# teofum/rust_raytracer

Hardware: AMD Instinct MI355X
Metric: Msamples/sec (whole node), cornell_dragon 870k tri @1000spp (higher is better)
Workload: dtype f64; 1 GPU; scenes/cornell_dragon 1200x1200 @1000spp (10 replicas x 10x10 strata), 871200-tri stand-in mesh; spp=1000, seed=1, pipeline=auto, frames_in_flight=1, partition=1200-row bands round-robin over 1 GPU(s)

## Files before the change

### rust_raytracer_amd/csrc/rt_bvh.cpp

```cpp
#include "rt_bvh.h"

#include <algorithm>
#include <cmath>
#include <cstdlib>
#include <limits>

#include "rt_refit.h"
#include "rt_scene.h"

namespace rt {
namespace {

constexpr int kMaxBins = 64;
static int g_bins = 16;
constexpr double kInf = std::numeric_limits<double>::infinity();

struct Box {
    double lo[3] = {kInf, kInf, kInf};
    double hi[3] = {-kInf, -kInf, -kInf};
    void grow(const double* p) {
        for (int a = 0; a < 3; a++) {
            if (p[a] < lo[a]) lo[a] = p[a];
            if (p[a] > hi[a]) hi[a] = p[a];
        }
// ... 228 lines not shown
Bvh4Build collapse_bvh4(const BvhBuild& b2) { return collapse<4>(b2); }



ConeLimits cone_limits(bool f32) {
    if (f32) return ConeLimits{1.0 / 32.0, 1e-12, 1e12};
    return ConeLimits{1.0 / 1048576.0, 1e-100, 1e100};
}

void build_mesh_cones(const std::vector<BuildNode4>& nodes4, const std::vector<TriRec<double>>& tris, const ConeLimits& lim,
                      std::vector<uint32_t>* out) {
    const size_t n_tris = tris.size();
    std::vector<double> normal(3 * n_tris);
    const double kNaN = std::numeric_limits<double>::quiet_NaN();
    for (size_t t = 0; t < n_tris; t++) rf_tri_normal(tris[t].v0, tris[t].e1, tris[t].e2, lim, &normal[3 * t]);
    struct Below {
        uint32_t lo = UINT32_MAX, hi = 0, count = 0;
        double sum[3] = {0.0, 0.0, 0.0};
        void add(const Below& o) {
            lo = std::min(lo, o.lo); hi = std::max(hi, o.hi); count += o.count;
            for (int a = 0; a < 3; a++) sum[a] += o.sum[a];
        }
    };
    auto cone_word = [&](const Below& b) -> uint32_t { return rf_cone_word(normal.data(), b.lo, b.hi, b.count, b.sum); };
    out->assign(4 * nodes4.size(), kNeutralCone);
    std::vector<Below> below(nodes4.size());
    for (size_t i = nodes4.size(); i-- > 0;) {
        const BuildNode4& nd = nodes4[i];
        Below all;
        for (int k = 0; k < 4; k++) {
            const int32_t ch = nd.child[k];
            if (ch == kEmptyChild) continue;
            Below b;
            if (ch >= 0) {
                if (size_t(ch) <= i || size_t(ch) >= nodes4.size()) { all.sum[0] = kNaN; continue; }
                b = below[size_t(ch)];
            } else {
                const uint32_t code = uint32_t(~ch), first = code >> 3, count = (code & 7u) + 1u;
                if (size_t(first) + count > n_tris) { all.sum[0] = kNaN; continue; }
                b.lo = first; b.hi = first + count; b.count = count;
                for (uint32_t t = first; t < first + count; t++)
                    for (int a = 0; a < 3; a++) b.sum[a] += normal[3 * size_t(t) + a];
            }
            (*out)[4 * i + size_t(k)] = cone_word(b);
            all.add(b);
        }
        below[i] = all;
    }
}

void build_mesh_slabs(const std::vector<BuildNode4>& nodes4, const std::vector<TriRec<double>>& tris, const std::vector<uint32_t>& cones,
                      const BvhNode4q* qnodes, const double* node_pad, std::vector<uint32_t>* out) {
    const size_t n_tris = tris.size();
    struct Run { uint32_t lo = UINT32_MAX, hi = 0, count = 0; };
    auto tri_at = [&](uint32_t t, double* v) {
        const TriRec<double>& r = tris[t];
        for (int a = 0; a < 3; a++) { v[a] = r.v0[a]; v[3 + a] = r.e1[a]; v[6 + a] = r.e2[a]; }
    };
    out->assign(4 * nodes4.size(), kNeutralSlab);
    std::vector<Run> below(nodes4.size());
    for (size_t i = nodes4.size(); i-- > 0;) {
        const BuildNode4& nd = nodes4[i];
        Run all;
        for (int k = 0; k < 4; k++) {
            const int32_t ch = nd.child[k];
            if (ch == kEmptyChild) continue;
            Run b;
            if (ch >= 0) {
                if (size_t(ch) <= i || size_t(ch) >= nodes4.size()) continue;
                b = below[size_t(ch)];
            } else {
                const uint32_t code = uint32_t(~ch), first = code >> 3, count = (code & 7u) + 1u;
                if (size_t(first) + count > n_tris) continue;
                b.lo = first; b.hi = first + count; b.count = count;
            }
            (*out)[4 * i + size_t(k)] = rf_slab_word(cones[4 * i + size_t(k)], qnodes[i].org, qnodes[i].cell, node_pad[i], b.lo, b.hi, b.count, tri_at);
            all.lo = std::min(all.lo, b.lo); all.hi = std::max(all.hi, b.hi);
            all.count += b.count;
        }
        below[i] = all;
    }
}

}
```

### rust_raytracer_amd/csrc/rt_bvh.h

```cpp
#pragma once
#include <cstdint>
#include <string>
#include <vector>

#include "rt_scene.h"

namespace rt {

struct BuildNode {
    double lo0[3], hi0[3], lo1[3], hi1[3];
    int32_t c0, c1;
};

struct BvhBuild {
    std::vector<BuildNode> nodes;
    std::vector<uint32_t> tri_order;
    uint32_t max_depth = 0;
};

BvhBuild build_bvh(const double* positions, const uint32_t* tri_pos, uint32_t n_tris, uint32_t max_leaf);

bool build_bvh_device(const double* positions, uint32_t n_positions, const uint32_t* tri_pos, uint32_t n_tris, uint32_t max_leaf,
                      BvhBuild* out, std::string* err);

template <int W>
struct BuildNodeN {
    double lo[W][3], hi[W][3];
    int32_t child[W];
};
template <int W>
struct BvhNBuild {
    std::vector<BuildNodeN<W>> nodes;
    uint32_t max_depth = 0;
    uint32_t max_stack = 0;
    double root_lo[3], root_hi[3];
};
using BuildNode4 = BuildNodeN<4>;
using Bvh4Build = BvhNBuild<4>;
Bvh4Build collapse_bvh4(const BvhBuild& bvh2);

struct ConeLimits {
    double sigma;
    double min_edge;
    double max_edge;
};
ConeLimits cone_limits(bool f32);
void build_mesh_cones(const std::vector<BuildNode4>& nodes4, const std::vector<TriRec<double>>& tris, const ConeLimits& lim,
                      std::vector<uint32_t>* out);
void build_mesh_slabs(const std::vector<BuildNode4>& nodes4, const std::vector<TriRec<double>>& tris, const std::vector<uint32_t>& cones,
                      const BvhNode4q* qnodes, const double* node_pad, std::vector<uint32_t>* out);

}
```

### rust_raytracer_amd/csrc/rt_refit.h

```cpp
#pragma once
#include <cmath>
#include <cstdint>
#include <cstring>
#include <limits>
#include <string>
#include <vector>

#include "../../include/rt_mi355.h"
#include "rt_bvh.h"
#include "rt_scene.h"

#if defined(__HIP__)
#include <hip/hip_runtime.h>

#include "rt_owned.h"
#define RT_HD __host__ __device__
#else
#define RT_HD
#endif

namespace rt {

RT_HD inline double rf_min(double a, double b) { return b < a ? b : a; }
RT_HD inline double rf_max(double a, double b) { return b > a ? b : a; }
// ... 85 lines not shown
            uint32_t ql = 255u, qh = 0u;
            if (any && real[k]) {
                const double l = std::floor((flo[k] - org) / cell), h = std::ceil((fhi[k] - org) / cell);
                const double lc = 255.0 < l ? 255.0 : l, hc = 255.0 < h ? 255.0 : h;
                ql = uint32_t(0.0 < lc ? lc : 0.0);
                qh = uint32_t(0.0 < hc ? hc : 0.0);
                if (!(org + ql * cell <= flo[k] && org + qh * cell >= fhi[k])) return false;
            }
            qlo[a] |= ql << (8 * k);
            qhi[a] |= qh << (8 * k);
        }
    }
    return true;
}

constexpr double kConeDirSlack = 0.00682;
constexpr double kConeSafety = 0.001;
constexpr double kConeMinCos = 0.125;

RT_HD inline void rf_tri_normal(const double* v0, const double* a, const double* b, const ConeLimits& lim, double* out) {
    const double cx = a[1] * b[2] - a[2] * b[1], cy = a[2] * b[0] - a[0] * b[2], cz = a[0] * b[1] - a[1] * b[0];
    const double la = std::sqrt(a[0] * a[0] + a[1] * a[1] + a[2] * a[2]), lb = std::sqrt(b[0] * b[0] + b[1] * b[1] + b[2] * b[2]);
    const double lc = std::sqrt(cx * cx + cy * cy + cz * cz);
    bool ok = std::isfinite(v0[0]) && std::isfinite(v0[1]) && std::isfinite(v0[2]);
    ok = ok && la >= lim.min_edge && la <= lim.max_edge && lb >= lim.min_edge && lb <= lim.max_edge;
    ok = ok && lc >= lim.sigma * la * lb && lc > 0.0;
    const double kNaN = std::numeric_limits<double>::quiet_NaN();
    out[0] = ok ? cx / lc : kNaN;
    out[1] = ok ? cy / lc : kNaN;
    out[2] = ok ? cz / lc : kNaN;
}

RT_HD inline uint32_t rf_cone_around(const double* normal, uint32_t lo, uint32_t hi, const double* axis) {
    const double l = std::sqrt(axis[0] * axis[0] + axis[1] * axis[1] + axis[2] * axis[2]);
    if (!(l > 0.0) || !std::isfinite(l)) return kNeutralCone;
    int q[3];
    double al = 0.0;
    for (int a = 0; a < 3; a++) { q[a] = int(std::lround(127.0 * axis[a] / l)); al += double(q[a]) * double(q[a]); }
    al = std::sqrt(al);
    if (!(al > 0.0)) return kNeutralCone;
    const double ax = q[0] / al, ay = q[1] / al, az = q[2] / al;
    double c = 1.0;
    for (uint32_t t = lo; t < hi; t++) {
        const double d = ax * normal[3 * size_t(t)] + ay * normal[3 * size_t(t) + 1] + az * normal[3 * size_t(t) + 2];
        c = d < c ? d : c;
        if (c < kConeMinCos) return kNeutralCone;
    }
    if (!(c >= kConeMinCos)) return kNeutralCone;
    const double s = std::sqrt(std::fmax(0.0, 1.0 - c * c));
    const double w = std::ceil(al * (s + kConeDirSlack + kConeSafety));
    if (!(w >= 1.0 && w <= 127.0)) return kNeutralCone;
    return uint32_t(q[0] & 0xFF) | (uint32_t(q[1] & 0xFF) << 8) | (uint32_t(q[2] & 0xFF) << 16) | (uint32_t(w) << 24);
}

RT_HD inline uint32_t rf_cone_word(const double* normal, uint32_t lo, uint32_t hi, uint32_t count, const double* sum) {
    if (count == 0 || hi - lo != count) return kNeutralCone;
    uint32_t word = rf_cone_around(normal, lo, hi, sum);
    if (word == kNeutralCone && count >= 2 && count <= 8 && std::isfinite(sum[0])) {
        uint32_t bi = lo, bj = lo;
        double least = 2.0;
        for (uint32_t i = lo; i < hi; i++)
            for (uint32_t j = i + 1; j < hi; j++) {
                const double* ni = &normal[3 * size_t(i)];
                const double* nj = &normal[3 * size_t(j)];
                const double dij = ni[0] * nj[0] + ni[1] * nj[1] + ni[2] * nj[2];
                if (dij < least) { least = dij; bi = i; bj = j; }
            }
        const double mid[3] = {normal[3 * size_t(bi)] + normal[3 * size_t(bj)], normal[3 * size_t(bi) + 1] + normal[3 * size_t(bj) + 1],
                               normal[3 * size_t(bi) + 2] + normal[3 * size_t(bj) + 2]};
        word = rf_cone_around(normal, lo, hi, mid);
    }
    return word;
}

RT_HD inline double rf_slab_inv_scale(const float* cell) {
    const double cmax = rf_max(double(cell[0]), rf_max(double(cell[1]), double(cell[2])));
    return 0.25 / cmax;
}
RT_HD inline double rf_slab_margin(const int* q, double pad, double inv_s) {
    const double l1 = double((q[0] < 0 ? -q[0] : q[0]) + (q[1] < 0 ? -q[1] : q[1]) + (q[2] < 0 ? -q[2] : q[2]));
    return l1 * (2.0 * pad * inv_s + 1.0 / 4096.0);
}

template <typename TriAt>
RT_HD inline uint32_t rf_slab_word(uint32_t cone, const float* org, const float* cell, double pad, uint32_t lo, uint32_t hi, uint32_t count, TriAt tri_at) {
    if (cone == kNeutralCone || count == 0 || hi - lo != count) return kNeutralSlab;
    const int q[3] = {int(int8_t(cone & 0xFFu)), int(int8_t((cone >> 8) & 0xFFu)), int(int8_t((cone >> 16) & 0xFFu))};
    const double inv_s = rf_slab_inv_scale(cell);
    if (!(inv_s > 0.0) || !std::isfinite(inv_s) || !std::isfinite(pad)) return kNeutralSlab;
    double plo = INFINITY, phi = -INFINITY;
    for (uint32_t t = lo; t < hi; t++) {
        double v[9];
        tri_at(t, v);
        for (int c = 0; c < 3; c++) {
            double x[3];
            for (int a = 0; a < 3; a++) x[a] = c == 0 ? v[a] : v[a] + v[3 * c + a];
            const double p = double(q[0]) * ((x[0] - double(org[0])) * inv_s) + double(q[1]) * ((x[1] - double(org[1])) * inv_s) +
                             double(q[2]) * ((x[2] - double(org[2])) * inv_s);
            plo = rf_min(plo, p);
            phi = rf_max(phi, p);
        }
    }
    if (!(plo <= phi) || !std::isfinite(plo) || !std::isfinite(phi)) return kNeutralSlab;
    const double margin = rf_slab_margin(q, pad, inv_s);
    const double l = rf_max(std::floor(plo - margin), -32768.0), h = rf_min(std::ceil(phi + margin), 32767.0);
    if (!(l <= 32767.0 && h >= -32768.0)) return kNeutralSlab;
    return (uint32_t(int32_t(l)) & 0xFFFFu) | (uint32_t(int32_t(h)) << 16);
}

#if defined(__HIP__)
struct RefitMesh {
    uint32_t n_tris = 0, n_nodes = 0, n_nodes4 = 0, n_positions = 0, n_normals = 0, n_uvs = 0;
    DevBuf<uint32_t> tri_order, tri_pos, tri_nrm;
    DevBuf<int32_t> tri_uv;
    DevBuf<int32_t> child2, child4;
    DevBuf<int32_t> parent2, parent4;
    DevBuf<uint32_t> inner2, inner4;
    DevBuf<uint32_t> arrived2, arrived4;
    DevBuf<double> positions, normals, uvs;
    DevBuf<double> tri_box, tri_normal;
    DevBuf<double> box2, box4;
    DevBuf<double> sum4;
    DevBuf<uint32_t> run4;
};

template <typename R>
struct RefitTarget {
    BvhNode<R>* nodes;
    BvhNode4f* nodes4;
    MeshNode4qc* nodes4q;
    TriRec<R>* tris;
    TriAttr<R>* attrs;
    double pad4;
};

bool refit_mesh_upload(RefitMesh& rm, const RtMesh& m, const uint32_t* tri_order, const int32_t* child2, uint32_t n_nodes, const int32_t* child4,
                       uint32_t n_nodes4, hipStream_t stream, uint64_t* bytes, std::string* err);
template <typename R> bool refit_mesh_launch(RefitMesh& rm, const RefitTarget<R>& t, hipStream_t stream, std::string* err);
#endif

}
```

### rust_raytracer_amd/csrc/rt_refit.hip

```cpp
#include "rt_refit.h"

#include <algorithm>

namespace rt {
namespace {

#define REFIT_TRY(expr)                                                                 \
    do {                                                                                \
        hipError_t e_ = (expr);                                                         \
        if (e_ != hipSuccess) {                                                         \
            *err = std::string("scene refit: ") + hipGetErrorString(e_) + " at " #expr; \
            return false;                                                               \
        }                                                                               \
    } while (0)

template <typename R>
__global__ void k_refit_tris(uint32_t n, const uint32_t* __restrict__ tri_order, const uint32_t* __restrict__ tri_pos,
                             const uint32_t* __restrict__ tri_nrm, const int32_t* __restrict__ tri_uv, const double* __restrict__ positions,
                             const double* __restrict__ normals, const double* __restrict__ uvs, ConeLimits lim, TriRec<R>* __restrict__ tris,
                             TriAttr<R>* __restrict__ attrs, double* __restrict__ tri_box, double* __restrict__ tri_normal) {
    const uint32_t slot = blockIdx.x * blockDim.x + threadIdx.x;
    if (slot >= n) return;
    const size_t t = tri_order[slot];
    const double* p0 = positions + 3 * size_t(tri_pos[3 * t]);
// ... 82 lines not shown
        if (W == 4) {
            for (int a = 0; a < 3; a++) sum[3 * (W * size_t(i) + k) + a] = s[a];
            run[3 * (W * size_t(i) + k)] = rlo; run[3 * (W * size_t(i) + k) + 1] = rhi; run[3 * (W * size_t(i) + k) + 2] = cnt;
        }
    }
}

template <int W>
__global__ void k_refit_up(uint32_t n_nodes, uint32_t n_tris, const int32_t* __restrict__ child, const int32_t* __restrict__ parent,
                           const uint32_t* __restrict__ inner, unsigned int* __restrict__ arrived, const double* __restrict__ tri_box,
                           const double* __restrict__ tri_normal, double* box, double* sum, uint32_t* run) {
    const uint32_t first = blockIdx.x * blockDim.x + threadIdx.x;
    if (first >= n_nodes || inner[first] != 0u) return;
    int32_t node = int32_t(first);
    for (uint32_t guard = 0; guard <= n_nodes; guard++) {
        refit_node<W>(uint32_t(node), n_nodes, n_tris, child, tri_box, tri_normal, box, sum, run);
        __threadfence();
        const int32_t up = parent[node];
        if (up < 0 || uint32_t(up) >= n_nodes) return;
        if (atomicAdd(&arrived[up], 1u) + 1u < inner[up]) return;
        __threadfence();
        node = up;
    }
}

template <typename R>
__global__ void k_refit_nodes2(uint32_t n_nodes, const double* __restrict__ box, BvhNode<R>* __restrict__ nodes) {
    const uint32_t i = blockIdx.x * blockDim.x + threadIdx.x;
    if (i >= n_nodes) return;
    BvhNode<R>& n = nodes[i];
    const double* b0 = box + 12 * size_t(i);
    const double* b1 = b0 + 6;
    for (int a = 0; a < 3; a++) {
        rf_pad_box2<R>(b0[a], b0[3 + a], &n.lo0[a], &n.hi0[a]);
        rf_pad_box2<R>(b1[a], b1[3 + a], &n.lo1[a], &n.hi1[a]);
    }
}

__global__ void k_refit_nodes4(uint32_t n_nodes, double pad, const int32_t* __restrict__ child, const double* __restrict__ box,
                               const double* __restrict__ sum, const uint32_t* __restrict__ run, const double* __restrict__ tri_normal,
                               const uint32_t* __restrict__ tri_order, const uint32_t* __restrict__ tri_pos, const double* __restrict__ positions,
                               BvhNode4f* __restrict__ nodes4, MeshNode4qc* __restrict__ nodes4q) {
    const uint32_t i = blockIdx.x * blockDim.x + threadIdx.x;
    if (i >= n_nodes) return;
    double lo[4][3], hi[4][3];
    int32_t ch[4];
    for (int k = 0; k < 4; k++) {
        ch[k] = child[4 * size_t(i) + k];
        for (int a = 0; a < 3; a++) { lo[k][a] = box[6 * (4 * size_t(i) + k) + a]; hi[k][a] = box[6 * (4 * size_t(i) + k) + 3 + a]; }
    }
    BvhNode4f& f = nodes4[i];
    for (int k = 0; k < 4; k++) {
        rf_pad_box4f(lo[k][0], hi[k][0], pad, &f.lox[k], &f.hix[k]);
        rf_pad_box4f(lo[k][1], hi[k][1], pad, &f.loy[k], &f.hiy[k]);
        rf_pad_box4f(lo[k][2], hi[k][2], pad, &f.loz[k], &f.hiz[k]);
    }
    float org[3] = {0.f, 0.f, 0.f}, cell[3] = {0.f, 0.f, 0.f};
    uint32_t qlo[3], qhi[3];
    MeshNode4qc& q = nodes4q[i];
    if (rf_quantise4(lo, hi, ch, pad, org, cell, qlo, qhi))
        for (int a = 0; a < 3; a++) { q.node.org[a] = org[a]; q.node.cell[a] = cell[a]; q.node.qlo[a] = qlo[a]; q.node.qhi[a] = qhi[a]; }
    for (int k = 0; k < 4; k++) {
        uint32_t word = kNeutralCone;
        if (ch[k] != kEmptyChild) {
            const uint32_t* r = run + 3 * (4 * size_t(i) + k);
            word = rf_cone_word(tri_normal, r[0], r[1], r[2], sum + 3 * (4 * size_t(i) + k));
        }
        q.cones.word[k] = word;
        uint32_t slab = kNeutralSlab;
        if (word != kNeutralCone) {
            const uint32_t* r = run + 3 * (4 * size_t(i) + k);
            slab = rf_slab_word(word, org, cell, pad, r[0], r[1], r[2], [&](uint32_t slot, double* v) {
                const size_t t = tri_order[slot];
                const double* p0 = positions + 3 * size_t(tri_pos[3 * t]);
                const double* p1 = positions + 3 * size_t(tri_pos[3 * t + 1]);
                const double* p2 = positions + 3 * size_t(tri_pos[3 * t + 2]);
                for (int a = 0; a < 3; a++) { v[a] = p0[a]; v[3 + a] = p1[a] - p0[a]; v[6 + a] = p2[a] - p0[a]; }
            });
        }
        q.slabs.word[k] = slab;
    }
}

template <typename T>
bool dev_alloc(DevBuf<T>& p, size_t n, std::string* err) {
    if (p.reserve(std::max<size_t>(n, 1) * sizeof(T)) == RT_OK) return true;
    *err = "scene refit: " + g_err;
    return false;
}
template <typename T>
bool dev_put(DevBuf<T>& dst, const T* src, size_t n, hipStream_t stream, uint64_t* bytes, std::string* err) {
    if (n) REFIT_TRY(hipMemcpyAsync(dst, src, n * sizeof(T), hipMemcpyHostToDevice, stream));
    *bytes += n * sizeof(T);
    return true;
}

inline dim3 grid_for(uint32_t n) { return dim3((n + 255u) / 256u); }

}

bool refit_mesh_upload(RefitMesh& rm, const RtMesh& m, const uint32_t* tri_order, const int32_t* child2, uint32_t n_nodes, const int32_t* child4,
                       uint32_t n_nodes4, hipStream_t stream, uint64_t* bytes, std::string* err) {
    if (!rm.tri_order) {
        RefitMesh r;
        r.n_tris = m.n_triangles; r.n_nodes = n_nodes; r.n_nodes4 = n_nodes4;
        r.n_positions = m.n_positions; r.n_normals = m.n_normals; r.n_uvs = m.uvs && m.tri_uv ? m.n_uvs : 0;
        const size_t nt = r.n_tris;
        bool ok = dev_alloc(r.tri_order, nt, err) && dev_alloc(r.tri_pos, 3 * nt, err) && dev_alloc(r.tri_nrm, 3 * nt, err) &&
                  (!m.tri_uv || dev_alloc(r.tri_uv, 3 * nt, err)) && dev_alloc(r.child2, 2 * size_t(n_nodes), err) &&
                  dev_alloc(r.child4, 4 * size_t(n_nodes4), err) && dev_alloc(r.parent2, n_nodes, err) && dev_alloc(r.parent4, n_nodes4, err) &&
                  dev_alloc(r.inner2, n_nodes, err) && dev_alloc(r.inner4, n_nodes4, err) && dev_alloc(r.arrived2, n_nodes, err) &&
                  dev_alloc(r.arrived4, n_nodes4, err) && dev_alloc(r.positions, 3 * size_t(r.n_positions), err) &&
                  dev_alloc(r.normals, 3 * size_t(r.n_normals), err) && (!r.n_uvs || dev_alloc(r.uvs, 3 * size_t(r.n_uvs), err)) &&
                  dev_alloc(r.tri_box, 6 * nt, err) && dev_alloc(r.tri_normal, 3 * nt, err) && dev_alloc(r.box2, 12 * size_t(n_nodes), err) &&
                  dev_alloc(r.box4, 24 * size_t(n_nodes4), err) && dev_alloc(r.sum4, 12 * size_t(n_nodes4), err) &&
                  dev_alloc(r.run4, 12 * size_t(n_nodes4), err);
        ok = ok && dev_put(r.tri_order, tri_order, nt, stream, bytes, err) && dev_put(r.tri_pos, m.tri_pos, 3 * nt, stream, bytes, err) &&
             dev_put(r.tri_nrm, m.tri_nrm, 3 * nt, stream, bytes, err) && (!m.tri_uv || dev_put(r.tri_uv, m.tri_uv, 3 * nt, stream, bytes, err)) &&
             dev_put(r.child2, child2, 2 * size_t(n_nodes), stream, bytes, err) && dev_put(r.child4, child4, 4 * size_t(n_nodes4), stream, bytes, err);
        if (!ok) return false;
        hipLaunchKernelGGL(k_refit_parents<2>, grid_for(n_nodes), dim3(256), 0, stream, n_nodes, r.child2.get(), r.parent2.get(), r.inner2.get());
        hipLaunchKernelGGL(k_refit_parents<4>, grid_for(n_nodes4), dim3(256), 0, stream, n_nodes4, r.child4.get(), r.parent4.get(), r.inner4.get());
        hipError_t e = hipGetLastError();
        if (e == hipSuccess) e = hipStreamSynchronize(stream);
        if (e != hipSuccess) { *err = std::string("scene refit: ") + hipGetErrorString(e); return false; }
        rm = std::move(r);
    }
    if (rm.n_tris != m.n_triangles || rm.n_positions != m.n_positions || rm.n_normals != m.n_normals || rm.n_nodes != n_nodes || rm.n_nodes4 != n_nodes4) {
        *err = "scene refit: the mesh has another structure than at its first update";
        return false;
    }
    return dev_put(rm.positions, m.positions, 3 * size_t(rm.n_positions), stream, bytes, err) &&
           dev_put(rm.normals, m.normals, 3 * size_t(rm.n_normals), stream, bytes, err) &&
           (!rm.n_uvs || dev_put(rm.uvs, m.uvs, 3 * size_t(rm.n_uvs), stream, bytes, err));
}

template <typename R>
bool refit_mesh_launch(RefitMesh& rm, const RefitTarget<R>& t, hipStream_t stream, std::string* err) {
    if (rm.n_tris == 0) return true;
    const dim3 block(256);
    REFIT_TRY(hipMemsetAsync(rm.arrived2, 0, size_t(rm.n_nodes) * sizeof(uint32_t), stream));
    REFIT_TRY(hipMemsetAsync(rm.arrived4, 0, size_t(rm.n_nodes4) * sizeof(uint32_t), stream));
    hipLaunchKernelGGL((k_refit_tris<R>), grid_for(rm.n_tris), block, 0, stream, rm.n_tris, rm.tri_order.get(), rm.tri_pos.get(), rm.tri_nrm.get(), rm.uvs ? rm.tri_uv.get() : nullptr,
                       rm.positions.get(), rm.normals.get(), rm.uvs.get(), cone_limits(sizeof(R) == 4), t.tris, t.attrs, rm.tri_box.get(), rm.tri_normal.get());
    hipLaunchKernelGGL((k_refit_up<2>), grid_for(rm.n_nodes), block, 0, stream, rm.n_nodes, rm.n_tris, rm.child2.get(), rm.parent2.get(), rm.inner2.get(), rm.arrived2.get(),
                       rm.tri_box.get(), rm.tri_normal.get(), rm.box2.get(), static_cast<double*>(nullptr), static_cast<uint32_t*>(nullptr));
    hipLaunchKernelGGL((k_refit_up<4>), grid_for(rm.n_nodes4), block, 0, stream, rm.n_nodes4, rm.n_tris, rm.child4.get(), rm.parent4.get(), rm.inner4.get(), rm.arrived4.get(),
                       rm.tri_box.get(), rm.tri_normal.get(), rm.box4.get(), rm.sum4.get(), rm.run4.get());
    hipLaunchKernelGGL((k_refit_nodes2<R>), grid_for(rm.n_nodes), block, 0, stream, rm.n_nodes, rm.box2.get(), t.nodes);
    hipLaunchKernelGGL(k_refit_nodes4, grid_for(rm.n_nodes4), block, 0, stream, rm.n_nodes4, t.pad4, rm.child4.get(), rm.box4.get(), rm.sum4.get(), rm.run4.get(),
                       rm.tri_normal.get(), rm.tri_order.get(), rm.tri_pos.get(), rm.positions.get(), t.nodes4, t.nodes4q);
    REFIT_TRY(hipGetLastError());
    return true;
}
template bool refit_mesh_launch<float>(RefitMesh&, const RefitTarget<float>&, hipStream_t, std::string*);
template bool refit_mesh_launch<double>(RefitMesh&, const RefitTarget<double>&, hipStream_t, std::string*);

}
```

### rust_raytracer_amd/csrc/rt_tables.cpp

```cpp
#include "rt_tables.h"

#include <algorithm>
#include <cmath>

#include "rt_refit.h"

namespace rt {

static int refuse(std::string* err, const char* msg) {
    if (err) *err = msg;
    return RT_E_UNSUPPORTED;
}

double mesh_pad(const CompiledScene& cs, const CompiledScene::MeshGeom& g) {
    double pad = 0.0;
    for (size_t i = 0; i < cs.meshes.size(); i++)
        if (cs.meshes[i].node4_base == g.node4_base) pad = std::fmax(pad, rf_pad_of_box(cs.mesh_bounds[i].lo, cs.mesh_bounds[i].hi));
    return pad;
}

template <typename R> static void derive_nodes2(const CompiledScene& cs, std::vector<BvhNode<R>>* out) {
    out->resize(cs.nodes.size());
    for (size_t i = 0; i < out->size(); i++) {
        const BuildNode& s = cs.nodes[i];
        BvhNode<R>& n = (*out)[i];
        for (int a = 0; a < 3; a++) {
            rf_pad_box2<R>(s.lo0[a], s.hi0[a], &n.lo0[a], &n.hi0[a]);
            rf_pad_box2<R>(s.lo1[a], s.hi1[a], &n.lo1[a], &n.hi1[a]);
        }
        n.c0 = s.c0;
        n.c1 = s.c1;
    }
}

static std::vector<double> derive_node_pads(const CompiledScene& cs) {
    std::vector<double> pad(cs.nodes4.size(), 0.0);
    for (const CompiledScene::MeshGeom& g : cs.mesh_geoms) std::fill_n(pad.begin() + g.node4_base, g.n_nodes4, mesh_pad(cs, g));
    return pad;
}

static void derive_nodes4f(const CompiledScene& cs, const std::vector<double>& node_pad, std::vector<BvhNode4f>* out) {
    out->resize(cs.nodes4.size());
    for (size_t i = 0; i < out->size(); i++) {
        const BuildNode4& sn = cs.nodes4[i];
        BvhNode4f& dn = (*out)[i];
        for (int k = 0; k < 4; k++) {
            float* lo[3] = {&dn.lox[k], &dn.loy[k], &dn.loz[k]};
            float* hi[3] = {&dn.hix[k], &dn.hiy[k], &dn.hiz[k]};
            for (int a = 0; a < 3; a++) rf_pad_box4f(sn.lo[k][a], sn.hi[k][a], node_pad[i], lo[a], hi[a]);
            dn.child[k] = sn.child[k];
            dn._pad[k] = 0;
        }
    }
}

static bool quantise(const BuildNode4& sn, double m, BvhNode4q& qn) {
    for (int k = 0; k < 4; k++) qn.child[k] = sn.child[k];
    return rf_quantise4(sn.lo, sn.hi, sn.child, m, qn.org, qn.cell, qn.qlo, qn.qhi);
}

static int derive_nodes4qc(const CompiledScene& cs, const std::vector<double>& node_pad, bool f32, std::vector<MeshNode4qc>* out, std::string* err) {
    std::vector<BvhNode4q> nodes4q(cs.nodes4.size());
    for (size_t i = 0; i < nodes4q.size(); i++)
        if (!quantise(cs.nodes4[i], node_pad[i], nodes4q[i])) return refuse(err, "BVH node does not fit the 8-bit grid");
    std::vector<uint32_t> cone_words, slab_words;
    build_mesh_cones(cs.nodes4, cs.tris, cone_limits(f32), &cone_words);
    build_mesh_slabs(cs.nodes4, cs.tris, cone_words, nodes4q.data(), node_pad.data(), &slab_words);
    out->resize(cs.nodes4.size());
    for (size_t i = 0; i < out->size(); i++) {
        MeshNode4qc& n = (*out)[i];
        n.node = nodes4q[i];
        for (int k = 0; k < 4; k++) n.cones.word[k] = cone_words[4 * i + size_t(k)];
        for (int k = 0; k < 4; k++) n.slabs.word[k] = slab_words[4 * i + size_t(k)];
        for (uint32_t& x : n._pad) x = 0;
    }
    return RT_OK;
}

template <typename R> static void derive_triangles(const CompiledScene& cs, std::vector<TriRec<R>>* tris, std::vector<TriAttr<R>>* attrs) {
    tris->resize(cs.tris.size());
    for (size_t i = 0; i < tris->size(); i++) {
        TriRec<R>& t = (*tris)[i];
        cast_arr(t.v0, cs.tris[i].v0); cast_arr(t.e1, cs.tris[i].e1); cast_arr(t.e2, cs.tris[i].e2);
        t._pad = R(0);
    }
    attrs->resize(cs.attrs.size());
    for (size_t i = 0; i < attrs->size(); i++) {
        const auto& s = cs.attrs[i];
        TriAttr<R>& a = (*attrs)[i];
        cast_arr(a.n0, s.n0); cast_arr(a.n1, s.n1); cast_arr(a.n2, s.n2);
        cast_arr(a.uv0, s.uv0); cast_arr(a.uv1, s.uv1); cast_arr(a.uv2, s.uv2);
        a.has_uv = s.has_uv;
        a._pad = 0;
    }
}

template <typename R>
int derive_mesh_tables(const CompiledScene& cs, MeshTables<R>* out, std::string* err) {
    *out = MeshTables<R>{};
    const std::vector<double> node_pad = derive_node_pads(cs);
    derive_nodes2(cs, &out->nodes);
    derive_nodes4f(cs, node_pad, &out->nodes4);
    if (int st = derive_nodes4qc(cs, node_pad, sizeof(R) == 4, &out->nodes4qc, err)) return st;
    derive_triangles(cs, &out->tris, &out->attrs);
    return RT_OK;
}

template <typename R> static void derive_prims(const CompiledScene& cs, SceneTables<R>* t) {
    t->bounds.resize(cs.bounds.size());
    for (size_t i = 0; i < t->bounds.size(); i++) {
        cast_arr(t->bounds[i].lo, cs.bounds[i].lo);
        cast_arr(t->bounds[i].hi, cs.bounds[i].hi);
    }
    t->xforms.resize(cs.xforms.size());
    for (size_t i = 0; i < t->xforms.size(); i++) {
        cast_arr(t->xforms[i].m, cs.xforms[i].m);
        cast_arr(t->xforms[i].inv, cs.xforms[i].inv);
    }
    t->spheres.resize(cs.spheres.size());
    for (size_t i = 0; i < t->spheres.size(); i++) {
        cast_arr(t->spheres[i].center, cs.spheres[i].center);
        t->spheres[i].radius = R(cs.spheres[i].radius);
        t->spheres[i].material = cs.spheres[i].material;
        t->spheres[i]._pad = 0;
    }
    t->planes.resize(cs.planes.size());
    for (size_t i = 0; i < t->planes.size(); i++) {
        const auto& s = cs.planes[i];
        PlanePrim<R>& p = t->planes[i];
        cast_arr(p.corner, s.corner); cast_arr(p.normal, s.normal);
        cast_arr(p.u, s.u); cast_arr(p.v, s.v);
        cast_arr(p.inv_u, s.inv_u); cast_arr(p.inv_v, s.inv_v);
        p.area = R(s.area);
        p.material = s.material;
        p.backface = s.backface;
    }
    t->suns.resize(cs.suns.size());
    for (size_t i = 0; i < t->suns.size(); i++) {
        cast_arr(t->suns[i].direction, cs.suns[i].direction);
        t->suns[i].material = cs.suns[i].material;
        t->suns[i]._pad = 0;
    }
    t->volumes.resize(cs.volumes.size());
    for (size_t i = 0; i < t->volumes.size(); i++) {
        t->volumes[i].neg_inv_density = R(cs.volumes[i].neg_inv_density);
        t->volumes[i].material = cs.volumes[i].material;
        t->volumes[i]._pad = 0;
    }
}
// ... 124 lines not shown
```

Before: 1587 Msamples/s.

## Add oriented slab axes to BVH4 children lacking normal cones

For BVH4 child slots that have no usable normal cone, the build now projects the child's triangles onto 46 fixed oblique axes. It picks the axis whose extent is smallest relative to the AABB, and only if that ratio is below a threshold, then stores it as a slab-only word with a quantised slab interval. A matching GPU refit kernel recomputes the choice after refit. The aim is to cull more ray-box hits with a tighter oriented slab test, in exchange for extra build and refit work. The traversal code that consumes slab-only words is not shown here.

```diff
diff --git a/rust_raytracer_amd/csrc/rt_bvh.cpp b/rust_raytracer_amd/csrc/rt_bvh.cpp
--- a/rust_raytracer_amd/csrc/rt_bvh.cpp
+++ b/rust_raytracer_amd/csrc/rt_bvh.cpp
@@ -334,4 +334,121 @@
     }
 }
 
-}
+bool slab_axes_enabled() {
+    const char* e = std::getenv("RT_SLAB_AXES");
+    return !(e && *e && std::atoi(e) == 0);
+}
+
+namespace {
+struct AxisSupport {
+    double lo[kSlabAxes], hi[kSlabAxes];
+    AxisSupport() { for (int c = 0; c < kSlabAxes; c++) { lo[c] = INFINITY; hi[c] = -INFINITY; } }
+    void merge(const AxisSupport& o) { for (int c = 0; c < kSlabAxes; c++) { lo[c] = rf_min(lo[c], o.lo[c]); hi[c] = rf_max(hi[c], o.hi[c]); } }
+};
+
+struct AxisPass {
+    const std::vector<BuildNode4>& nodes4;
+    const std::vector<TriRec<double>>& tris;
+    const BvhNode4q* qnodes;
+    const double* node_pad;
+    std::vector<uint32_t>& cones;
+    struct Run { uint32_t lo = UINT32_MAX, hi = 0, count = 0; };
+    std::vector<Run> run;
+    std::vector<uint8_t> eligible;
+    std::vector<uint8_t> done;
+    double ax[kSlabAxes], ay[kSlabAxes], az[kSlabAxes];
+
+    void project(uint32_t lo, uint32_t hi, AxisSupport* s) const {
+        double mn[kSlabAxes], mx[kSlabAxes];
+        for (int c = 0; c < kSlabAxes; c++) { mn[c] = s->lo[c]; mx[c] = s->hi[c]; }
+        for (uint32_t t = lo; t < hi; t++) {
+            const TriRec<double>& r = tris[t];
+            double v[9];
+            for (int a = 0; a < 3; a++) { v[a] = r.v0[a]; v[3 + a] = r.e1[a]; v[6 + a] = r.e2[a]; }
+            for (int c3 = 0; c3 < 3; c3++) {
+                double x[3];
+                rf_tri_corner(v, c3, x);
+                const double x0 = x[0], x1 = x[1], x2 = x[2];
+                for (int c = 0; c < kSlabAxes; c++) {
+                    const double p = ax[c] * x0 + ay[c] * x1 + az[c] * x2;
+                    mn[c] = p < mn[c] ? p : mn[c];
+                    mx[c] = p > mx[c] ? p : mx[c];
+                }
+            }
+        }
+        for (int c = 0; c < kSlabAxes; c++) { s->lo[c] = mn[c]; s->hi[c] = mx[c]; }
+    }
+    void visit(size_t i, int k, AxisSupport* s) {
+        const size_t id = 4 * i + size_t(k), c = size_t(nodes4[i].child[k]);
+        done[id] = 1;
+        for (int j = 0; j < 4; j++) {
+            if (nodes4[c].child[j] == kEmptyChild) continue;
+            if (eligible[4 * c + size_t(j)]) {
+                AxisSupport below;
+                visit(c, j, &below);
+                s->merge(below);
+            } else {
+                project(run[4 * c + size_t(j)].lo, run[4 * c + size_t(j)].hi, s);
+            }
+        }
+        const int pick = rf_slab_axis_pick(nodes4[i].lo[k], nodes4[i].hi[k], s->lo, s->hi);
+        if (pick < 0) return;
+        const uint32_t word = rf_slab_axis_word(pick);
+        const Run& r = run[id];
+        const uint32_t slab = rf_slab_word(word, qnodes[i].org, qnodes[i].cell, node_pad[i], r.lo, r.hi, r.count, [&](uint32_t t, double* v) {
+            for (int a = 0; a < 3; a++) { v[a] = tris[t].v0[a]; v[3 + a] = tris[t].e1[a]; v[6 + a] = tris[t].e2[a]; }
+        });
+        if (slab != kNeutralSlab) cones[id] = word;
+    }
+};
+}
+
+void build_mesh_slab_axes(const std::vector<BuildNode4>& nodes4, const std::vector<TriRec<double>>& tris, const ConeLimits& lim,
+                          const BvhNode4q* qnodes, const double* node_pad, std::vector<uint32_t>* cones) {
+    const size_t n = nodes4.size(), n_tris = tris.size();
+    if (n == 0 || cones->size() != 4 * n) return;
+    AxisPass p{nodes4, tris, qnodes, node_pad, *cones, {}, {}, {}, {}, {}, {}};
+    for (int c = 0; c < kSlabAxes; c++) {
+        int q[3];
+        rf_slab_axis(c, q);
+        p.ax[c] = double(q[0]); p.ay[c] = double(q[1]); p.az[c] = double(q[2]);
+    }
+    std::vector<uint32_t> bad_before(n_tris + 1, 0);
+    for (size_t t = 0; t < n_tris; t++) {
+        double nrm[3];
+        rf_tri_normal(tris[t].v0, tris[t].e1, tris[t].e2, lim, nrm);
+        bad_before[t + 1] = bad_before[t] + (std::isfinite(nrm[0]) ? 0u : 1u);
+    }
+    p.run.resize(4 * n);
+    p.eligible.assign(4 * n, 0);
+    p.done.assign(4 * n, 0);
+    for (size_t i = n; i-- > 0;) {
+        for (int k = 0; k < 4; k++) {
+            const int32_t ch = nodes4[i].child[k];
+            AxisPass::Run& b = p.run[4 * i + size_t(k)];
+            if (ch == kEmptyChild) continue;
+            if (ch >= 0) {
+                if (size_t(ch) <= i || size_t(ch) >= n) continue;
+                for (int j = 0; j < 4; j++) {
+                    const AxisPass::Run& o = p.run[4 * size_t(ch) + size_t(j)];
+                    b.lo = std::min(b.lo, o.lo); b.hi = std::max(b.hi, o.hi); b.count += o.count;
+                }
+                if (b.count == 0 || b.hi - b.lo != b.count || b.hi > n_tris) continue;
+                const double clean[3] = {bad_before[b.hi] == bad_before[b.lo] ? 0.0 : std::numeric_limits<double>::quiet_NaN(), 0.0, 0.0};
+                p.eligible[4 * i + size_t(k)] = rf_slab_axis_eligible(0, 1, (*cones)[4 * i + size_t(k)], b.lo, b.hi, b.count, clean) ? 1 : 0;
+            } else {
+                const uint32_t code = uint32_t(~ch), first = code >> 3, count = (code & 7u) + 1u;
+                if (size_t(first) + count > n_tris) continue;
+                b.lo = first; b.hi = first + count; b.count = count;
+            }
+        }
+    }
+    for (size_t i = 0; i < n; i++)
+        for (int k = 0; k < 4; k++)
+            if (p.eligible[4 * i + size_t(k)] && !p.done[4 * i + size_t(k)]) {
+                AxisSupport s;
+                p.visit(i, k, &s);
+            }
+}
+
+}
diff --git a/rust_raytracer_amd/csrc/rt_bvh.h b/rust_raytracer_amd/csrc/rt_bvh.h
--- a/rust_raytracer_amd/csrc/rt_bvh.h
+++ b/rust_raytracer_amd/csrc/rt_bvh.h
@@ -47,6 +47,8 @@
 ConeLimits cone_limits(bool f32);
 void build_mesh_cones(const std::vector<BuildNode4>& nodes4, const std::vector<TriRec<double>>& tris, const ConeLimits& lim,
                       std::vector<uint32_t>* out);
+void build_mesh_slab_axes(const std::vector<BuildNode4>& nodes4, const std::vector<TriRec<double>>& tris, const ConeLimits& lim,
+                          const BvhNode4q* qnodes, const double* node_pad, std::vector<uint32_t>* cones);
 void build_mesh_slabs(const std::vector<BuildNode4>& nodes4, const std::vector<TriRec<double>>& tris, const std::vector<uint32_t>& cones,
                       const BvhNode4q* qnodes, const double* node_pad, std::vector<uint32_t>* out);
 
diff --git a/rust_raytracer_amd/csrc/rt_refit.h b/rust_raytracer_amd/csrc/rt_refit.h
--- a/rust_raytracer_amd/csrc/rt_refit.h
+++ b/rust_raytracer_amd/csrc/rt_refit.h
@@ -191,10 +191,29 @@
     return l1 * (2.0 * pad * inv_s + 1.0 / 4096.0);
 }
 
+RT_HD inline void rf_cone_axis(uint32_t cone, int* q) {
+    q[0] = int(int8_t(cone & 0xFFu)); q[1] = int(int8_t((cone >> 8) & 0xFFu)); q[2] = int(int8_t((cone >> 16) & 0xFFu));
+}
+RT_HD inline void rf_tri_corner(const double* v, int c, double* x) {
+    for (int a = 0; a < 3; a++) x[a] = c == 0 ? v[a] : v[a] + v[3 * c + a];
+}
+RT_HD inline double rf_slab_project(const int* q, const float* org, double inv_s, const double* x) {
+    return double(q[0]) * ((x[0] - double(org[0])) * inv_s) + double(q[1]) * ((x[1] - double(org[1])) * inv_s) +
+           double(q[2]) * ((x[2] - double(org[2])) * inv_s);
+}
+RT_HD inline uint32_t rf_slab_finish(const int* q, double pad, double inv_s, double plo, double phi) {
+    if (!(plo <= phi) || !std::isfinite(plo) || !std::isfinite(phi)) return kNeutralSlab;
+    const double margin = rf_slab_margin(q, pad, inv_s);
+    const double l = rf_max(std::floor(plo - margin), -32768.0), h = rf_min(std::ceil(phi + margin), 32767.0);
+    if (!(l <= 32767.0 && h >= -32768.0)) return kNeutralSlab;
+    return (uint32_t(int32_t(l)) & 0xFFFFu) | (uint32_t(int32_t(h)) << 16);
+}
+
 template <typename TriAt>
 RT_HD inline uint32_t rf_slab_word(uint32_t cone, const float* org, const float* cell, double pad, uint32_t lo, uint32_t hi, uint32_t count, TriAt tri_at) {
     if (cone == kNeutralCone || count == 0 || hi - lo != count) return kNeutralSlab;
-    const int q[3] = {int(int8_t(cone & 0xFFu)), int(int8_t((cone >> 8) & 0xFFu)), int(int8_t((cone >> 16) & 0xFFu))};
+    int q[3];
+    rf_cone_axis(cone, q);
     const double inv_s = rf_slab_inv_scale(cell);
     if (!(inv_s > 0.0) || !std::isfinite(inv_s) || !std::isfinite(pad)) return kNeutralSlab;
     double plo = INFINITY, phi = -INFINITY;
@@ -203,19 +222,74 @@
         tri_at(t, v);
         for (int c = 0; c < 3; c++) {
             double x[3];
-            for (int a = 0; a < 3; a++) x[a] = c == 0 ? v[a] : v[a] + v[3 * c + a];
-            const double p = double(q[0]) * ((x[0] - double(org[0])) * inv_s) + double(q[1]) * ((x[1] - double(org[1])) * inv_s) +
-                             double(q[2]) * ((x[2] - double(org[2])) * inv_s);
+            rf_tri_corner(v, c, x);
+            const double p = rf_slab_project(q, org, inv_s, x);
             plo = rf_min(plo, p);
             phi = rf_max(phi, p);
         }
     }
-    if (!(plo <= phi) || !std::isfinite(plo) || !std::isfinite(phi)) return kNeutralSlab;
-    const double margin = rf_slab_margin(q, pad, inv_s);
-    const double l = rf_max(std::floor(plo - margin), -32768.0), h = rf_min(std::ceil(phi + margin), 32767.0);
-    if (!(l <= 32767.0 && h >= -32768.0)) return kNeutralSlab;
-    return (uint32_t(int32_t(l)) & 0xFFFFu) | (uint32_t(int32_t(h)) << 16);
-}
+    return rf_slab_finish(q, pad, inv_s, plo, phi);
+}
+
+#ifndef RT_SLAB_AXIS_COUNT
+#define RT_SLAB_AXIS_COUNT 46
+#endif
+#ifndef RT_SLAB_AXIS_MAX_RATIO
+#define RT_SLAB_AXIS_MAX_RATIO 0.9
+#endif
+constexpr int kSlabAxes = RT_SLAB_AXIS_COUNT;
+static_assert(kSlabAxes >= 1 && kSlabAxes <= 46, "a prefix of the table");
+constexpr double kSlabAxisMaxRatio = RT_SLAB_AXIS_MAX_RATIO;
+RT_HD inline void rf_slab_axis(int c, int* q) {
+    static constexpr int8_t kTable[46][3] = {
+        {0, 89, -89},   {0, 89, 89},    {89, -89, 0},   {89, 0, -89},    {89, 0, 89},    {89, 89, 0},    {72, -72, -72},  {72, -72, 72},
+        {72, 72, -72},  {72, 72, 72},   {0, 56, -112},  {0, 56, 112},    {0, 112, -56},  {0, 112, 56},   {56, -112, 0},   {56, 0, -112},
+        {56, 0, 112},   {56, 112, 0},   {112, -56, 0},  {112, 0, -56},   {112, 0, 56},   {112, 56, 0},   {42, -84, -84},  {51, -102, -51},
+        {51, -102, 51}, {42, -84, 84},  {51, -51, -102}, {51, -51, 102}, {51, 51, -102}, {51, 51, 102},  {42, 84, -84},   {51, 102, -51},
+        {51, 102, 51},  {42, 84, 84},   {84, -84, -42}, {84, -84, 42},   {84, -42, -84}, {102, -51, -51}, {102, -51, 51}, {84, -42, 84},
+        {84, 42, -84},  {102, 51, -51}, {102, 51, 51},  {84, 42, 84},    {84, 84, -42},  {84, 84, 42}};
+    q[0] = kTable[c][0]; q[1] = kTable[c][1]; q[2] = kTable[c][2];
+}
+RT_HD inline double rf_axis_project(const int* q, const double* x) { return double(q[0]) * x[0] + double(q[1]) * x[1] + double(q[2]) * x[2]; }
+
+RT_HD inline bool rf_slab_axis_eligible(int32_t ch, uint32_t n_nodes, uint32_t cone, uint32_t lo, uint32_t hi, uint32_t count, const double* sum) {
+    if (ch < 0 || uint32_t(ch) >= n_nodes || cone != kNeutralCone) return false;
+    if (count == 0 || hi - lo != count) return false;
+    return std::isfinite(sum[0]) && std::isfinite(sum[1]) && std::isfinite(sum[2]);
+}
+
+RT_HD inline int rf_slab_axis_pick(const double* blo, const double* bhi, const double* smin, const double* smax) {
+    double ext[3];
+    for (int a = 0; a < 3; a++) {
+        ext[a] = bhi[a] - blo[a];
+        if (!(ext[a] > 0.0) || !std::isfinite(ext[a])) return -1;
+    }
+    int best = -1;
+    double best_ratio = kSlabAxisMaxRatio;
+    for (int c = 0; c < kSlabAxes; c++) {
+        int q[3];
+        rf_slab_axis(c, q);
+        const double den = double(q[0] < 0 ? -q[0] : q[0]) * ext[0] + double(q[1] < 0 ? -q[1] : q[1]) * ext[1] + double(q[2] < 0 ? -q[2] : q[2]) * ext[2];
+        const double num = smax[c] - smin[c];
+        if (!(num >= 0.0) || !std::isfinite(num) || !(den > 0.0) || !std::isfinite(den)) return -1;
+        const double ratio = num / den;
+        if (ratio < best_ratio) { best_ratio = ratio; best = c; }
+    }
+    return best;
+}
+RT_HD inline uint32_t rf_slab_axis_word(int c) {
+    int q[3];
+    rf_slab_axis(c, q);
+    return uint32_t(q[0] & 0xFF) | (uint32_t(q[1] & 0xFF) << 8) | (uint32_t(q[2] & 0xFF) << 16) | (127u << 24);
+}
+RT_HD inline bool rf_is_slab_only(uint32_t cone) {
+    int q[3];
+    rf_cone_axis(cone, q);
+    const int l2 = q[0] * q[0] + q[1] * q[1] + q[2] * q[2];
+    return (cone >> 24) == 127u && l2 > 0 && l2 <= 126 * 126;
+}
+
+bool slab_axes_enabled();
 
 #if defined(__HIP__)
 struct RefitMesh {
diff --git a/rust_raytracer_amd/csrc/rt_refit.hip b/rust_raytracer_amd/csrc/rt_refit.hip
--- a/rust_raytracer_amd/csrc/rt_refit.hip
+++ b/rust_raytracer_amd/csrc/rt_refit.hip
@@ -188,6 +188,115 @@
     }
 }
 
+constexpr int kAxisGroup = 8;
+constexpr int kAxisBlock = 256;
+constexpr int kAxisWaves = kAxisBlock / 64;
+
+__device__ inline double wave_min(double v) {
+    for (int off = 32; off >= 1; off >>= 1) v = rf_min(v, __shfl_xor(v, off, 64));
+    return v;
+}
+__device__ inline double wave_max(double v) {
+    for (int off = 32; off >= 1; off >>= 1) v = rf_max(v, __shfl_xor(v, off, 64));
+    return v;
+}
+
+__global__ __launch_bounds__(kAxisBlock) void k_refit_slab_axes(uint32_t n_nodes, double pad, const int32_t* __restrict__ child, const double* __restrict__ box,
+                                                                const double* __restrict__ sum, const uint32_t* __restrict__ run,
+                                                                const uint32_t* __restrict__ tri_order, const uint32_t* __restrict__ tri_pos,
+                                                                const double* __restrict__ positions, MeshNode4qc* __restrict__ nodes4q) {
+    const size_t id = blockIdx.x;
+    const size_t i = id >> 2;
+    const int k = int(id & 3u);
+    if (i >= n_nodes) return;
+    const uint32_t lo = run[3 * id], hi = run[3 * id + 1], count = run[3 * id + 2];
+    if (!rf_slab_axis_eligible(child[id], n_nodes, nodes4q[i].cones.word[k], lo, hi, count, sum + 3 * id)) return;
+    __shared__ double s_lo[kAxisWaves][kSlabAxes], s_hi[kAxisWaves][kSlabAxes];
+    __shared__ double s_p[kAxisWaves][2];
+    __shared__ int s_pick;
+    const int tid = int(threadIdx.x), wave = tid >> 6, lane = tid & 63;
+    auto corners = [&](uint32_t slot, double* v) {
+        const size_t t = tri_order[slot];
+        const double* p0 = positions + 3 * size_t(tri_pos[3 * t]);
+        const double* p1 = positions + 3 * size_t(tri_pos[3 * t + 1]);
+        const double* p2 = positions + 3 * size_t(tri_pos[3 * t + 2]);
+        for (int a = 0; a < 3; a++) { v[a] = p0[a]; v[3 + a] = p1[a] - p0[a]; v[6 + a] = p2[a] - p0[a]; }
+    };
+    for (int g = 0; g < kSlabAxes; g += kAxisGroup) {
+        int q[kAxisGroup][3];
+        double mn[kAxisGroup], mx[kAxisGroup];
+#pragma unroll
+        for (int c = 0; c < kAxisGroup; c++) {
+            rf_slab_axis(g + c < kSlabAxes ? g + c : kSlabAxes - 1, q[c]);
+            mn[c] = INFINITY;
+            mx[c] = -INFINITY;
+        }
+        for (uint32_t slot = lo + uint32_t(tid); slot < hi; slot += uint32_t(kAxisBlock)) {
+            double v[9];
+            corners(slot, v);
+            for (int c3 = 0; c3 < 3; c3++) {
+                double x[3];
+                rf_tri_corner(v, c3, x);
+#pragma unroll
+                for (int c = 0; c < kAxisGroup; c++) {
+                    const double p = rf_axis_project(q[c], x);
+                    mn[c] = rf_min(mn[c], p);
+                    mx[c] = rf_max(mx[c], p);
+                }
+            }
+        }
+#pragma unroll
+        for (int c = 0; c < kAxisGroup; c++) {
+            const double a = wave_min(mn[c]), b = wave_max(mx[c]);
+            if (lane == 0 && g + c < kSlabAxes) { s_lo[wave][g + c] = a; s_hi[wave][g + c] = b; }
+        }
+    }
+    __syncthreads();
+    if (tid == 0) {
+        double smin[kSlabAxes], smax[kSlabAxes];
+        for (int c = 0; c < kSlabAxes; c++) {
+            smin[c] = s_lo[0][c];
+            smax[c] = s_hi[0][c];
+            for (int w = 1; w < kAxisWaves; w++) { smin[c] = rf_min(smin[c], s_lo[w][c]); smax[c] = rf_max(smax[c], s_hi[w][c]); }
+        }
+        s_pick = rf_slab_axis_pick(box + 6 * id, box + 6 * id + 3, smin, smax);
+    }
+    __syncthreads();
+    const int pick = s_pick;
+    if (pick < 0) return;
+    const uint32_t word = rf_slab_axis_word(pick);
+    int q[3];
+    rf_cone_axis(word, q);
+    float org[3], cell[3];
+    for (int a = 0; a < 3; a++) { org[a] = nodes4q[i].node.org[a]; cell[a] = nodes4q[i].node.cell[a]; }
+    const double inv_s = rf_slab_inv_scale(cell);
+    if (!(inv_s > 0.0) || !std::isfinite(inv_s) || !std::isfinite(pad)) return;
+    double plo = INFINITY, phi = -INFINITY;
+    for (uint32_t slot = lo + uint32_t(tid); slot < hi; slot += uint32_t(kAxisBlock)) {
+        double v[9];
+        corners(slot, v);
+        for (int c3 = 0; c3 < 3; c3++) {
+            double x[3];
+            rf_tri_corner(v, c3, x);
+            const double p = rf_slab_project(q, org, inv_s, x);
+            plo = rf_min(plo, p);
+            phi = rf_max(phi, p);
+        }
+    }
+    plo = wave_min(plo);
+    phi = wave_max(phi);
+    if (lane == 0) { s_p[wave][0] = plo; s_p[wave][1] = phi; }
+    __syncthreads();
+    if (tid == 0) {
+        for (int w = 1; w < kAxisWaves; w++) { plo = rf_min(plo, s_p[w][0]); phi = rf_max(phi, s_p[w][1]); }
+        const uint32_t slab = rf_slab_finish(q, pad, inv_s, plo, phi);
+        if (slab != kNeutralSlab) {
+            nodes4q[i].cones.word[k] = word;
+            nodes4q[i].slabs.word[k] = slab;
+        }
+    }
+}
+
 template <typename T>
 bool dev_alloc(DevBuf<T>& p, size_t n, std::string* err) {
     if (p.reserve(std::max<size_t>(n, 1) * sizeof(T)) == RT_OK) return true;
@@ -256,6 +365,9 @@
     hipLaunchKernelGGL((k_refit_nodes2<R>), grid_for(rm.n_nodes), block, 0, stream, rm.n_nodes, rm.box2.get(), t.nodes);
     hipLaunchKernelGGL(k_refit_nodes4, grid_for(rm.n_nodes4), block, 0, stream, rm.n_nodes4, t.pad4, rm.child4.get(), rm.box4.get(), rm.sum4.get(), rm.run4.get(),
                        rm.tri_normal.get(), rm.tri_order.get(), rm.tri_pos.get(), rm.positions.get(), t.nodes4, t.nodes4q);
+    if (slab_axes_enabled() && rm.n_nodes4 > 0)
+        hipLaunchKernelGGL(k_refit_slab_axes, dim3(4u * rm.n_nodes4), dim3(kAxisBlock), 0, stream, rm.n_nodes4, t.pad4, rm.child4.get(), rm.box4.get(), rm.sum4.get(),
+                           rm.run4.get(), rm.tri_order.get(), rm.tri_pos.get(), rm.positions.get(), t.nodes4q);
     REFIT_TRY(hipGetLastError());
     return true;
 }
diff --git a/rust_raytracer_amd/csrc/rt_tables.cpp b/rust_raytracer_amd/csrc/rt_tables.cpp
--- a/rust_raytracer_amd/csrc/rt_tables.cpp
+++ b/rust_raytracer_amd/csrc/rt_tables.cpp
@@ -65,6 +65,7 @@
         if (!quantise(cs.nodes4[i], node_pad[i], nodes4q[i])) return refuse(err, "BVH node does not fit the 8-bit grid");
     std::vector<uint32_t> cone_words, slab_words;
     build_mesh_cones(cs.nodes4, cs.tris, cone_limits(f32), &cone_words);
+    if (slab_axes_enabled()) build_mesh_slab_axes(cs.nodes4, cs.tris, cone_limits(f32), nodes4q.data(), node_pad.data(), &cone_words);
     build_mesh_slabs(cs.nodes4, cs.tris, cone_words, nodes4q.data(), node_pad.data(), &slab_words);
     out->resize(cs.nodes4.size());
     for (size_t i = 0; i < out->size(); i++) {
```

After: 1621 Msamples/s, median of 6. 2.1% higher.
